# aapdo/M3ViT

Measured on AMD Instinct MI355X. Metric: images/sec fwd+bwd ViT-S/16 MoE(E=16,k=4) 224^2 bs=128, higher is better.
Workload: dtype f16; 1 GPU; configs[1]: ViT-Small/16 + MoE E=16 top-k=4 multi_gate, synthetic 224x224; batch_per_gpu=128, global_batch=128, task_passes=2, launch=hipGraph replay (one linear graph per task pass and stream), routing=deterministic (std=0), task_streams=2, wgrad_streams=0, activation_checkpointing=False, parallelism=single, full=False

## Files before the change

### m3vit_amd/csrc/wgrad_dev.h

```cpp
#pragma once
#include "common.h"
#include <type_traits>

namespace m3 {

constexpr int WG_T = 128;
constexpr int WG_ROWS = 64;
constexpr int WG_THREADS = 256;
constexpr int BG_T = 256, BG_THREADS = 512, BG_RS = 512;

constexpr int WG_MULTI = 8;

struct WgradRdProb {
  const float *ws; float *dW; const float *bws; float *db;
  int64_t e4; int32_t b4;
  int32_t nbw;
  int32_t first;
  int32_t beta;
};

struct WgradDev {
  const char *dC; int64_t lddc_b; const int32_t *c_row_idx;
  int32_t c_row_div; const float *c_row_scale;
  int32_t a_row_sh, c_row_sh;
  const char *A; int64_t lda_b; const int32_t *a_row_idx; int32_t a_row_div;
  int64_t M; int32_t N; int32_t K; int32_t G;
  const int32_t *group_offsets;
  int32_t splits;
  float *ws;
  float *bias_ws;
  int32_t tiles_k;
  int32_t chunk_rows;
  int32_t rd_blocks, rd_zslices;
  int32_t rd_nbx, rd_nbw;
  int32_t rd_cols;
  const float *rd_ws; int32_t rd_splits; int64_t rd_e4;
  const int32_t *rd_off; int32_t rd_G, rd_chunk;
  float *rd_dW; int32_t rd_beta;
  const float *rd_bws; int64_t rd_b4; float *rd_db; int32_t rd_beta_db;
  int32_t rd_n;
  WgradRdProb rd_tab0, rd_tab1, rd_tab2, rd_tab3, rd_tab4, rd_tab5, rd_tab6, rd_tab7;
  float *direct_dW; float *direct_db; int32_t direct_beta, direct_beta_db;
  int32_t lpt;
};

__device__ __forceinline__ void wgrad_store_tile(const WgradDev &p, const f32x4 (&acc)[4][4], int64_t slab_id, int g, int n0, int k0,
                                                 int wr, int wc, int li, int lg) {
  float *out = p.direct_dW ? p.direct_dW + (int64_t)g * p.N * p.K : p.ws + slab_id * (int64_t)p.N * p.K;
  const bool add = p.direct_dW && p.direct_beta;
#pragma unroll
  for (int ni = 0; ni < 4; ++ni) {
    const int n = n0 + wc * 64 + ni * 16 + li;
    if (n >= p.N) continue;
    f32x4 old[4];
    if (add) {
#pragma unroll
      for (int ki = 0; ki < 4; ++ki) {
        const int k = k0 + wr * 64 + ki * 16 + 4 * lg;
        old[ki] = k < p.K ? *(const f32x4 *)(out + (int64_t)n * p.K + k) : f32x4{0.f, 0.f, 0.f, 0.f};
      }
    }
#pragma unroll
    for (int ki = 0; ki < 4; ++ki) {
      const int k = k0 + wr * 64 + ki * 16 + 4 * lg;
      if (k >= p.K) continue;
      *(f32x4 *)(out + (int64_t)n * p.K + k) = add ? acc[ki][ni] + old[ki] : acc[ki][ni];
    }
  }
}
__device__ __forceinline__ void wgrad_store_bias(const WgradDev &p, float v, int64_t slab_id, int g, int n) {
  if (p.direct_db) {
    float *d = p.direct_db + (int64_t)g * p.N + n;
    *d = p.direct_beta_db ? *d + v : v;
  } else {
    p.bias_ws[slab_id * p.N + n] = v;
  }
}

__host__ __device__ __forceinline__ int wgrad_units_of_group(int rows, int chunk) { return (rows + chunk - 1) / chunk; }
__host__ __device__ __forceinline__ void wgrad_unit_rows(int rows, int n, int j, int &begin, int &end) {
  const int per = ((rows + n - 1) / n + WG_ROWS - 1) / WG_ROWS * WG_ROWS;
  begin = j * per;
  end = begin + per < rows ? begin + per : rows;
}

__device__ __forceinline__ void wgrad_unit_scan(const int32_t *off, int G, int chunk, int lane, int &rows, int &n, int &first) {
  rows = lane < G ? off[lane + 1] - off[lane] : 0;
  n = wgrad_units_of_group(rows, chunk);
  int incl = n;
#pragma unroll
  for (int d = 1; d < 64; d <<= 1) {
    const int t = __shfl_up(incl, d, 64);
    if (lane >= d) incl += t;
  }
  first = incl - n;
}

__device__ __forceinline__ bool wgrad_unit(const int32_t *off, int G, int chunk, int lin, int tiles, int lane, int &tile,
                                           int &u, int &g, int64_t &r0, int64_t &r1) {
  int rows, n, first;
  wgrad_unit_scan(off, G, chunk, lane, rows, n, first);
  const int units = __shfl(first + n, 63, 64);
  if (lin >= units * tiles) return false;
  const int log_id = xcd_remap(lin, units * tiles);
  tile = log_id % tiles;
  u = log_id / tiles;
  const unsigned long long m = __ballot(u >= first && u < first + n);
  g = __ffsll((long long)m) - 1;
  rows = __shfl(rows, g, 64); n = __shfl(n, g, 64); first = __shfl(first, g, 64);
  int b, e;
  wgrad_unit_rows(rows, n, u - first, b, e);
  r0 = (int64_t)off[g] + b;
  r1 = (int64_t)off[g] + e;
  return true;
}

__device__ __forceinline__ int wgrad_lpt_group(const int32_t *off, int G, int u, int lane) {
  if (G > 64 || (G & 7)) return u;
  const int cnt = lane < G ? off[lane + 1] - off[lane] : -1;
  int rank = 0;
  for (int j = 0; j < G; ++j) {
    const int cj = __shfl(cnt, j, 64);
    rank += (cj > cnt || (cj == cnt && j < lane)) ? 1 : 0;
  }
  const int per = G >> 3;
  const int want = 8 * (u % per) + u / per;
  const unsigned long long m = __ballot(lane < G && rank == want);
  return __ffsll((long long)m) - 1;
}

struct WgradProb {
  const char *dC; int64_t lddc_b; const char *A; int64_t lda_b;
  float *ws; float *bias_ws;
  int32_t N, K, tiles_k;
  int32_t first;
};
struct WgradMultiDev {
  WgradDev d;
  WgradProb tab0, tab1, tab2, tab3, tab4, tab5, tab6, tab7;
};

typedef __fp16 fp16x4_t __attribute__((__vector_size__(4 * sizeof(__fp16))));

__device__ __forceinline__ f32x4 wgrad_sum_slabs(const f32x4 *w, int64_t elems4, int lo, int hi, f32x4 s) {
  int sp = lo;
  for (; sp + 8 <= hi; sp += 8) {
    f32x4 v[8];
#pragma unroll
    for (int j = 0; j < 8; ++j) v[j] = w[(int64_t)(sp + j) * elems4];
#pragma unroll
    for (int j = 0; j < 8; ++j) s += v[j];
  }
  for (; sp < hi; ++sp) s += w[(int64_t)sp * elems4];
  return s;
}
__device__ __forceinline__ void wgrad_reduce_block(int64_t blk, int tid, const float *ws, int splits, int64_t elems4, float *dW,
                                                   int beta, int nb_w, const float *bias_ws, int64_t belems4, float *db, int beta_db,
                                                   int cols) {
  if (blk >= nb_w) {
    blk -= nb_w; ws = bias_ws; elems4 = belems4; dW = db; beta = beta_db;
  }
  if (cols == 256) {
    const int64_t i = blk * 256 + tid;
    if (i >= elems4) return;
    f32x4 s = beta ? ((const f32x4 *)dW)[i] : f32x4{0.f, 0.f, 0.f, 0.f};
    ((f32x4 *)dW)[i] = wgrad_sum_slabs((const f32x4 *)ws + i, elems4, 0, splits, s);
    return;
  }
  __shared__ f32x4 spart[3][64];
  const int col = tid & 63, part = tid >> 6;
  const int64_t i = blk * 64 + col;
  const bool in = i < elems4;
  f32x4 s = f32x4{0.f, 0.f, 0.f, 0.f};
  if (in) {
    if (part == 0 && beta) s = ((const f32x4 *)dW)[i];
    s = wgrad_sum_slabs((const f32x4 *)ws + i, elems4, splits * part / 4, splits * (part + 1) / 4, s);
  }
  if (part > 0) spart[part - 1][col] = s;
  __syncthreads();
  if (part == 0 && in) {
    s += spart[0][col]; s += spart[1][col]; s += spart[2][col];
    ((f32x4 *)dW)[i] = s;
  }
}

__device__ __forceinline__ void wgrad_reduce_grouped_block(int64_t blk, int g, int tid, const float *ws, const int32_t *off, int G,
                                                           int chunk, int64_t elems4, float *dW, int beta, int nb_w,
                                                           const float *bias_ws, int64_t belems4, float *db, int beta_db) {
  if (blk >= nb_w) {
    blk -= nb_w; ws = bias_ws; elems4 = belems4; dW = db; beta = beta_db;
  }
  const int64_t i = blk * 256 + tid;
  int rows, n, first;
  wgrad_unit_scan(off, G, chunk, tid & 63, rows, n, first);
  n = __shfl(n, g, 64); first = __shfl(first, g, 64);
  if (i >= elems4) return;
  f32x4 *out = (f32x4 *)dW + (int64_t)g * elems4 + i;
  f32x4 s = beta ? *out : f32x4{0.f, 0.f, 0.f, 0.f};
  const f32x4 *w = (const f32x4 *)ws + (int64_t)first * elems4 + i;
  int u = 0;
  for (; u + 8 <= n; u += 8) {
    f32x4 v[8];
#pragma unroll
    for (int j = 0; j < 8; ++j) v[j] = w[(int64_t)(u + j) * elems4];
#pragma unroll
    for (int j = 0; j < 8; ++j) s += v[j];
  }
  if (u + 4 <= n) {
    f32x4 v[4];
#pragma unroll
    for (int j = 0; j < 4; ++j) v[j] = w[(int64_t)(u + j) * elems4];
#pragma unroll
    for (int j = 0; j < 4; ++j) s += v[j];
    u += 4;
  }
  if (u + 2 <= n) {
    const f32x4 v0 = w[(int64_t)u * elems4], v1 = w[(int64_t)(u + 1) * elems4];
    s += v0; s += v1;
    u += 2;
  }
  if (u < n) s += w[(int64_t)u * elems4];
  *out = s;
}

__device__ __forceinline__ bool wgrad_ride_along(const WgradDev &p, int tid, int &bz, int &gz) {
  bz = blockIdx.z; gz = gridDim.z;
  if (p.rd_blocks <= 0) return false;
  if (bz < p.rd_zslices) {
    const int rid = blockIdx.x + (int)gridDim.x * (blockIdx.y + (int)gridDim.y * bz);
    if (rid < p.rd_blocks) {
      const int g = rid / p.rd_nbx, bx = rid - g * p.rd_nbx;
      if (p.rd_n > 1) {
        const float *ws = p.rd_tab0.ws, *bws = p.rd_tab0.bws;
        float *dW = p.rd_tab0.dW, *db = p.rd_tab0.db;
        int64_t e4 = p.rd_tab0.e4;
        int b4 = p.rd_tab0.b4, nbw = p.rd_tab0.nbw, first = p.rd_tab0.first, beta = p.rd_tab0.beta;
#define M3_RD_FROM(j)                                                                                                   \
  {                                                                                                                     \
    const float *ws_ = p.rd_tab##j.ws, *bws_ = p.rd_tab##j.bws;                                                         \
    float *dW_ = p.rd_tab##j.dW, *db_ = p.rd_tab##j.db;                                                                 \
    const int64_t e4_ = p.rd_tab##j.e4;                                                                                 \
    const int b4_ = p.rd_tab##j.b4, nbw_ = p.rd_tab##j.nbw, first_ = p.rd_tab##j.first, beta_ = p.rd_tab##j.beta;       \
    const bool h_ = rid >= first_;                                                                                      \
    ws = h_ ? ws_ : ws; bws = h_ ? bws_ : bws; dW = h_ ? dW_ : dW; db = h_ ? db_ : db; e4 = h_ ? e4_ : e4;              \
    b4 = h_ ? b4_ : b4; nbw = h_ ? nbw_ : nbw; first = h_ ? first_ : first; beta = h_ ? beta_ : beta;                   \
  }
        static_assert(WG_MULTI == 8, "one M3_RD_FROM per entry");
        M3_RD_FROM(1) M3_RD_FROM(2) M3_RD_FROM(3) M3_RD_FROM(4) M3_RD_FROM(5) M3_RD_FROM(6) M3_RD_FROM(7)
#undef M3_RD_FROM
        wgrad_reduce_block(rid - first, tid, ws, p.rd_splits, e4, dW, beta & 1, nbw, bws, b4, db, beta >> 1, p.rd_cols);
      } else if (p.rd_chunk)
        wgrad_reduce_grouped_block(bx, g, tid, p.rd_ws, p.rd_off, p.rd_G, p.rd_chunk, p.rd_e4, p.rd_dW, p.rd_beta, p.rd_nbw,
                                   p.rd_bws, p.rd_b4, p.rd_db, p.rd_beta_db);
      else
        wgrad_reduce_block(bx, tid, p.rd_ws, p.rd_splits, p.rd_e4, p.rd_dW, p.rd_beta, p.rd_nbw, p.rd_bws, p.rd_b4, p.rd_db,
                           p.rd_beta_db, p.rd_cols);
    }
    return true;
  }
  bz -= p.rd_zslices; gz -= p.rd_zslices;
  return false;
}

template <typename T> __device__ __forceinline__ u32x4 scale_chunk(u32x4 v, float s);
template <> __device__ __forceinline__ u32x4 scale_chunk<half_t>(u32x4 v, float s) {
  f16x8 f = __builtin_bit_cast(f16x8, v);
#pragma unroll
  for (int j = 0; j < 8; ++j) f[j] = (half_t)((float)f[j] * s);
  return __builtin_bit_cast(u32x4, f);
}
template <> __device__ __forceinline__ u32x4 scale_chunk<bf16_t>(u32x4 v, float s) {
  bf16x8 f = __builtin_bit_cast(bf16x8, v);
#pragma unroll
  for (int j = 0; j < 8; ++j) f[j] = (bf16_t)((float)f[j] * s);
  return __builtin_bit_cast(u32x4, f);
}
template <> __device__ __forceinline__ u32x4 scale_chunk<float>(u32x4 v, float s) {
  return __builtin_bit_cast(u32x4, __builtin_bit_cast(f32x4, v) * s);
}

__device__ __forceinline__ f16x8 wgrad_tr16_frag(const char *p0, const char *p1) {
  typedef __attribute__((address_space(3))) fp16x4_t lds_h4;
  const fp16x4_t lo = __builtin_amdgcn_ds_read_tr16_b64_v4f16((lds_h4 *)p0);
  const fp16x4_t hi = __builtin_amdgcn_ds_read_tr16_b64_v4f16((lds_h4 *)p1);
  f16x8 f;
  f[0] = (half_t)lo[0]; f[1] = (half_t)lo[1]; f[2] = (half_t)lo[2]; f[3] = (half_t)lo[3];
  f[4] = (half_t)hi[0]; f[5] = (half_t)hi[1]; f[6] = (half_t)hi[2]; f[7] = (half_t)hi[3];
  return f;
}
template <typename T> __device__ __forceinline__ float wgrad_colsum8(const typename Mma<T>::frag &f, float a) {
  typedef T t2 __attribute__((ext_vector_type(2)));
  if constexpr (sizeof(T) == 4) {
    return a + ((f[0] + f[1]) + (f[2] + f[3]));
  } else {
#pragma unroll
    for (int j = 0; j < 4; ++j) {
      const t2 pr = t2{f[2 * j], f[2 * j + 1]};
      if constexpr (std::is_same<T, half_t>::value)
        a = __builtin_amdgcn_fdot2(pr, t2{(T)1, (T)1}, a, false);
      else if constexpr (std::is_same<T, bf16_t>::value)
        a = __builtin_amdgcn_fdot2_f32_bf16(pr, t2{(T)1.f, (T)1.f}, a, false);
    }
    return a;
  }
}
__device__ __forceinline__ f16x8 wgrad_factor_f16x8(f32x4 s0, f32x4 s1) {
  return f16x8{(half_t)s0[0], (half_t)s0[1], (half_t)s0[2], (half_t)s0[3], (half_t)s1[0], (half_t)s1[1], (half_t)s1[2], (half_t)s1[3]};
}

enum WgradKernel { WGRAD_STAGED, WGRAD_DMA, WGRAD_BIG, WGRAD_SKINNY };

template <typename T> constexpr int wgrad_dtype_of = std::is_same<T, half_t>::value ? M3_F16 : std::is_same<T, bf16_t>::value ? M3_BF16 : M3_F32;
template <typename Fam, typename T, int I = 0, typename F> static inline void wgrad_each_flags(F &f) {
  if constexpr (I < 8) {
    constexpr bool GC = (I & 1) != 0, GA = (I & 2) != 0, SC = (I & 4) != 0;
    if (const void *k = Fam::template instance<T, GC, GA, SC>()) f(wgrad_dtype_of<T>, GC, GA, SC, k);
    wgrad_each_flags<Fam, T, I + 1>(f);
  }
}
template <typename Fam, typename F> static inline void wgrad_each_instance(F f) {
  wgrad_each_flags<Fam, half_t>(f); wgrad_each_flags<Fam, bf16_t>(f); wgrad_each_flags<Fam, float>(f);
}
template <typename Fam>
static inline int wgrad_launch_instance(int dtype, bool gc, bool ga, bool sc, dim3 grid, dim3 block, size_t lds, WgradDev d, hipStream_t s) {
  const void *kernel = nullptr;
  wgrad_each_instance<Fam>([&](int dt, bool c, bool a, bool f, const void *k) { if (dt == dtype && c == gc && a == ga && f == sc) kernel = k; });
  M3_REQUIRE(kernel, "m3_wgrad_tn: no kernel instance for dtype %d, gathers (%d, %d), per-row factor %d", dtype, gc, ga, sc);
  void *args[] = {&d};
  (void)hipLaunchKernel(kernel, grid, block, args, lds, s);
  return check_launch("m3_wgrad_tn");
}

int launch_wgrad_staged(int dtype, bool gc, bool ga, bool sc, dim3 grid, const WgradDev &d, hipStream_t s);
int launch_wgrad_dma(int dtype, bool gc, bool ga, bool sc, dim3 grid, const WgradDev &d, hipStream_t s);
int launch_wgrad_big(int dtype, bool gc, bool ga, bool sc, dim3 grid, const WgradDev &d, hipStream_t s);
int launch_wgrad_multi(int dtype, dim3 grid, const WgradMultiDev &d, hipStream_t s);

}
```

### m3vit_amd/csrc/wgrad_staged.hip

```cpp
#include "wgrad_dev.h"

namespace m3 {

template <typename T> struct WgLds;
template <> struct WgLds<half_t> { static constexpr int STRIDE = 288; static constexpr int ROWS = 32; };
template <> struct WgLds<bf16_t> { static constexpr int STRIDE = 288; static constexpr int ROWS = 32; };
template <> struct WgLds<float> { static constexpr int STRIDE = 528; static constexpr int ROWS = 32; };

template <typename T>
__device__ __forceinline__ typename Mma<T>::frag read_tr_frag(const char *base, int rb, int col, int li, int lg);

template <>
__device__ __forceinline__ f16x8 read_tr_frag<half_t>(const char *base, int rb, int col, int li, int lg) {
  const char *p0 = base + (rb + 4 * lg + (li >> 2)) * WgLds<half_t>::STRIDE + (col + 4 * (li & 3)) * 2;
  const char *p1 = p0 + 16 * WgLds<half_t>::STRIDE;
  return wgrad_tr16_frag(p0, p1);
}

template <>
__device__ __forceinline__ bf16x8 read_tr_frag<bf16_t>(const char *base, int rb, int col, int li, int lg) {
  return __builtin_bit_cast(bf16x8, read_tr_frag<half_t>(base, rb, col, li, lg));
}

template <>
__device__ __forceinline__ f32x4 read_tr_frag<float>(const char *base, int rb, int col, int li, int lg) {
  const char *p = base + (rb + 4 * lg) * WgLds<float>::STRIDE + (col + li) * 4;
  f32x4 f;
  f[0] = *(const float *)(p);
  f[1] = *(const float *)(p + WgLds<float>::STRIDE);
  f[2] = *(const float *)(p + 2 * WgLds<float>::STRIDE);
  f[3] = *(const float *)(p + 3 * WgLds<float>::STRIDE);
  return f;
}

#ifdef M3_WGRAD_STAMPS
constexpr int WTSTAMP_WGS = 128, WTSTAMP_N = 2 + 4 * 80;
__device__ unsigned long long g_wtn_stamps[WTSTAMP_WGS][WTSTAMP_N];
#define WT_STAMP(i)                                                                                                   \
  do {                                                                                                                \
    const int wg_ = blockIdx.y + gridDim.y * blockIdx.z;                                                              \
    if (threadIdx.x == 0 && blockIdx.x == 0 && wg_ < WTSTAMP_WGS && (i) < WTSTAMP_N)                                  \
      g_wtn_stamps[wg_][(i)] = __builtin_amdgcn_s_memtime();                                                          \
  } while (0)
#else
#define WT_STAMP(i) do { } while (0)
#endif

template <typename T, bool GC, bool GA, bool SC>
__device__ __forceinline__ void wgrad_tile_loop(const WgradDev &p, int tile, int g, int64_t slab_id, int64_t r0, int64_t r1,
                                                int64_t s_begin, int nst) {
  typedef Mma<T> MM;
  typedef typename MM::frag frag;
  constexpr int ES = (int)sizeof(T);
  constexpr int EPC = 16 / ES;
  constexpr int STRIDE = WgLds<T>::STRIDE;
  constexpr int ROWS = WgLds<T>::ROWS;
  constexpr int CPR = WG_T * ES / 16;
  constexpr int NLD = ROWS * CPR / WG_THREADS;
  constexpr int RSTEP = WG_THREADS / CPR;
  constexpr int OPB = ROWS * STRIDE;
  constexpr int KCH = ROWS / MM::KC;

  extern __shared__ __attribute__((aligned(16))) char smem[];

  const int tid = threadIdx.x;
  const int lane = tid & 63, wave = tid >> 6;
  const int li = lane & 15, lg = lane >> 4;
  const int wr = wave >> 1, wc = wave & 1;

  const int tn = tile / p.tiles_k, tk = tile - tn * p.tiles_k;
  const int n0 = tn * WG_T, k0 = tk * WG_T;

  f32x4 acc[4][4];
#pragma unroll
  for (int a = 0; a < 4; ++a)
#pragma unroll
    for (int b = 0; b < 4; ++b) acc[a][b] = f32x4{0.f, 0.f, 0.f, 0.f};

  const int srow = tid / CPR, c = tid - srow * CPR;
  int ncol = n0 + c * EPC, kcol = k0 + c * EPC;
  if (ncol > p.N - EPC) ncol = p.N - EPC;
  if (kcol > p.K - EPC) kcol = p.K - EPC;
  const char *c_base = p.dC + (int64_t)ncol * ES;
  const char *a_base = p.A + (int64_t)kcol * ES;
  const int st_off = srow * STRIDE + c * 16;
  const uint32_t ldc = (uint32_t)p.lddc_b, lda = (uint32_t)p.lda_b;
  const uint32_t rbase = (uint32_t)(r0 + s_begin * ROWS + srow);
  const uint32_t rend = (uint32_t)r1;

  auto row_of = [&](int step, int i) -> uint32_t {
    const uint32_t m = rbase + (uint32_t)(step * ROWS + i * RSTEP);
    return m < rend ? m : rend - 1;
  };
  auto load_index = [&](int step, int32_t(&ic)[NLD], int32_t(&ia)[NLD]) {
#pragma unroll
    for (int i = 0; i < NLD; ++i) {
      const uint32_t m = row_of(step, i);
      if (GC) ic[i] = p.c_row_idx[m];
      if (GA) ia[i] = p.a_row_idx[m];
    }
  };
  auto load_global = [&](int step, const int32_t(&ic)[NLD], const int32_t(&ia)[NLD], u32x4(&rc)[NLD], u32x4(&ra)[NLD],
                         float(&rs)[NLD]) {
#pragma unroll
    for (int i = 0; i < NLD; ++i) {
      const uint32_t m = row_of(step, i);
      const uint32_t cr = GC ? (uint32_t)div_by(ic[i], p.c_row_div, p.c_row_sh) : m;
      const uint32_t ar = GA ? (uint32_t)div_by(ia[i], p.a_row_div, p.a_row_sh) : m;
      rc[i] = *(const u32x4 *)(c_base + (uint64_t)cr * ldc);
      ra[i] = *(const u32x4 *)(a_base + (uint64_t)ar * lda);
      if (SC) rs[i] = p.c_row_scale[ic[i]];
    }
  };
  auto store_lds = [&](int buf, int step, const u32x4(&rc)[NLD], const u32x4(&ra)[NLD], const float(&rs)[NLD]) {
    char *base = smem + buf * (2 * OPB) + st_off;
#pragma unroll
    for (int i = 0; i < NLD; ++i) {
      const bool ok = rbase + (uint32_t)(step * ROWS + i * RSTEP) < rend;
      const u32x4 cv = SC ? scale_chunk<T>(rc[i], rs[i]) : rc[i];
      *(u32x4 *)(base + i * RSTEP * STRIDE) = ok ? cv : u32x4{0u, 0u, 0u, 0u};
      *(u32x4 *)(base + i * RSTEP * STRIDE + OPB) = ok ? ra[i] : u32x4{0u, 0u, 0u, 0u};
    }
  };
  const bool do_bias = (p.bias_ws || p.direct_db) && tk == 0 && wr == 0;
  f32x4 acc_b[4];
#pragma unroll
  for (int i = 0; i < 4; ++i) acc_b[i] = f32x4{0.f, 0.f, 0.f, 0.f};
  frag ones;
#pragma unroll
  for (int j = 0; j < MM::EPL; ++j) ones[j] = (T)1.0f;

  auto compute = [&](int buf) {
    const char *sC = smem + buf * (2 * OPB), *sA = sC + OPB;
#pragma unroll
    for (int kc = 0; kc < KCH; ++kc) {
      frag fk[4], fn[4];
#pragma unroll
      for (int i = 0; i < 4; ++i) {
        fk[i] = read_tr_frag<T>(sA, kc * MM::KC, wr * 64 + i * 16, li, lg);
        fn[i] = read_tr_frag<T>(sC, kc * MM::KC, wc * 64 + i * 16, li, lg);
      }
#pragma unroll
      for (int ki = 0; ki < 4; ++ki)
#pragma unroll
        for (int ni = 0; ni < 4; ++ni) acc[ki][ni] = MM::mma(fk[ki], fn[ni], acc[ki][ni]);
      if (do_bias) {
#pragma unroll
        for (int ni = 0; ni < 4; ++ni) acc_b[ni] = MM::mma(ones, fn[ni], acc_b[ni]);
      }
    }
  };

  WT_STAMP(0);
  if (nst > 0) {
    const int last = nst - 1;
    auto cl = [&](int s_) { return s_ < last ? s_ : last; };
    u32x4 rc0[NLD], ra0[NLD], rc1[NLD], ra1[NLD];
    float sc0[NLD], sc1[NLD];
    int32_t ic0[NLD], ia0[NLD], ic1[NLD], ia1[NLD];
    auto fetch = [&](int ds, int32_t(&ic)[NLD], int32_t(&ia)[NLD], u32x4(&rc)[NLD], u32x4(&ra)[NLD], float(&rs)[NLD],
                     int32_t(&jc)[NLD], int32_t(&ja)[NLD]) {
      load_global(ds, ic, ia, rc, ra, rs);
#if defined(M3_WGRAD_STAMPS) && defined(M3_WGRAD_TN_INDEX_BEHIND)
      load_index(cl(ds + 1), jc, ja);
#else
      load_index(cl(ds + 2), ic, ia);
#endif
    };
    load_index(0, ic0, ia0);
    load_index(cl(1), ic1, ia1);
    load_global(0, ic0, ia0, rc1, ra1, sc1);
    load_index(cl(2), ic0, ia0);
    load_global(cl(1), ic1, ia1, rc0, ra0, sc0);
    load_index(cl(3), ic1, ia1);
    store_lds(0, 0, rc1, ra1, sc1);
    __syncthreads();
    WT_STAMP(1);
    int t = 0;
    for (; t + 3 < nst; t += 2) {
      fetch(t + 2, ic0, ia0, rc1, ra1, sc1, ic1, ia1);
      __builtin_amdgcn_sched_barrier(0);
      WT_STAMP(2 + 4 * t);
      compute(0);
      WT_STAMP(3 + 4 * t);
      store_lds(1, t + 1, rc0, ra0, sc0);
      WT_STAMP(4 + 4 * t);
      __syncthreads();
      WT_STAMP(5 + 4 * t);
      fetch(t + 3, ic1, ia1, rc0, ra0, sc0, ic0, ia0);
      __builtin_amdgcn_sched_barrier(0);
      WT_STAMP(6 + 4 * t);
      compute(1);
      WT_STAMP(7 + 4 * t);
      store_lds(0, t + 2, rc1, ra1, sc1);
      WT_STAMP(8 + 4 * t);
      __syncthreads();
      WT_STAMP(9 + 4 * t);
    }
    const int rem = nst - t;
    if (rem == 3) {
      load_global(t + 2, ic0, ia0, rc1, ra1, sc1);
      compute(0);
      store_lds(1, t + 1, rc0, ra0, sc0);
      __syncthreads();
      compute(1);
      store_lds(0, t + 2, rc1, ra1, sc1);
      __syncthreads();
      compute(0);
    } else if (rem == 2) {
      compute(0);
      store_lds(1, t + 1, rc0, ra0, sc0);
      __syncthreads();
      compute(1);
    } else {
      compute(0);
    }
  }

  if (do_bias && lg == 0) {
#pragma unroll
    for (int ni = 0; ni < 4; ++ni) {
      const int n = n0 + wc * 64 + ni * 16 + li;
      if (n < p.N) wgrad_store_bias(p, acc_b[ni][0], slab_id, g, n);
    }
  }
  wgrad_store_tile(p, acc, slab_id, g, n0, k0, wr, wc, li, lg);
}

template <typename T, bool GC, bool GA, bool SC = false>
__global__ __launch_bounds__(WG_THREADS, 2) void wgrad_tn_kernel(const WgradDev p) {
  constexpr int ROWS = WgLds<T>::ROWS;
  const int tid = threadIdx.x;
  const int lane = tid & 63;

  const int tiles = gridDim.x;
  int bz, gz;
  if (wgrad_ride_along(p, tid, bz, gz)) return;
  const int lin = blockIdx.x + tiles * (blockIdx.y + gridDim.y * bz);
  int tile, gs, g, sp, nst;
  int64_t r0, r1, s_begin;
  if (p.chunk_rows) {
    if (!wgrad_unit(p.group_offsets, p.G, p.chunk_rows, lin, tiles, lane, tile, gs, g, r0, r1)) return;
    sp = gs; s_begin = 0;
    nst = (int)((r1 - r0 + ROWS - 1) / ROWS);
  } else {
    const int log_id = xcd_remap(lin, tiles * gridDim.y * gz);
    tile = log_id % tiles; gs = log_id / tiles;
    g = gs % (int)gridDim.y; sp = gs / (int)gridDim.y;
    if (p.group_offsets && p.lpt) g = wgrad_lpt_group(p.group_offsets, p.G, g, lane);
    if (p.group_offsets) { r0 = p.group_offsets[g]; r1 = p.group_offsets[g + 1]; }
    else { r0 = 0; r1 = p.M; }
    const int64_t nsteps_all = (r1 - r0 + ROWS - 1) / ROWS;
    const int64_t per = (nsteps_all + p.splits - 1) / p.splits;
    s_begin = (int64_t)sp * per;
    int64_t s_end = s_begin + per;
    if (s_end > nsteps_all) s_end = nsteps_all;
    nst = (int)(s_end > s_begin ? s_end - s_begin : 0);
  }
  const int64_t slab_id = p.chunk_rows ? (int64_t)sp : (int64_t)sp * p.G + g;
  wgrad_tile_loop<T, GC, GA, SC>(p, tile, g, slab_id, r0, r1, s_begin, nst);
}

struct WgStaged {
  template <typename T, bool GC, bool GA, bool SC> static const void *instance() {
    if constexpr (!SC || GC) return (const void *)wgrad_tn_kernel<T, GC, GA, SC>;
    else return nullptr;
  }
};

int launch_wgrad_staged(int dtype, bool gc, bool ga, bool sc, dim3 grid, const WgradDev &d, hipStream_t s) {
  const size_t lds16 = 4 * WgLds<half_t>::ROWS * WgLds<half_t>::STRIDE, lds32 = 4 * WgLds<float>::ROWS * WgLds<float>::STRIDE;
  static bool attr_set = false;
  if (!attr_set) {
    wgrad_each_instance<WgStaged>([&](int dt, bool, bool, bool, const void *k) {
      (void)hipFuncSetAttribute(k, hipFuncAttributeMaxDynamicSharedMemorySize, (int)(dt == M3_F32 ? lds32 : lds16));
    });
    attr_set = true;
  }
  return wgrad_launch_instance<WgStaged>(dtype, gc, ga, sc, grid, dim3(WG_THREADS), dtype == M3_F32 ? lds32 : lds16, d, s);
}

}

#ifdef M3_WGRAD_STAMPS
extern "C" int m3_debug_wtn_stamps(unsigned long long *dst, int wgs, int clear) {
  using namespace m3;
  if (wgs > WTSTAMP_WGS) wgs = WTSTAMP_WGS;
  const size_t bytes = (size_t)wgs * WTSTAMP_N * sizeof(unsigned long long);
  if (dst && hipMemcpyFromSymbol(dst, HIP_SYMBOL(g_wtn_stamps), bytes) != hipSuccess) return M3_ERR_LAUNCH;
  if (clear) {
    void *sym = nullptr;
    if (hipGetSymbolAddress(&sym, HIP_SYMBOL(g_wtn_stamps)) != hipSuccess || hipMemset(sym, 0, sizeof(g_wtn_stamps)) != hipSuccess) return M3_ERR_LAUNCH;
  }
  return M3_OK;
}
#endif
```

Measured before the change: 7743 images/s.

## Stage gather row indices in an LDS table and advance ungathered row pointers incrementally

The staged weight-gradient kernel used to load row indices and scale factors from global memory every step, per thread and per loaded row. It now fetches them cooperatively in 256-row pieces, applies the divisor once, and writes them to a double-buffered LDS table. Later steps read this table, spreading the piece loads across a four-pair-of-steps schedule. For ungathered operands it advances precomputed pointers instead of recomputing row addresses and clamps. This cuts dependent global index latency and address arithmetic in the inner loop, at the cost of extra LDS, which may affect occupancy, and more code specialisation.

```diff
diff --git a/m3vit_amd/csrc/wgrad_dev.h b/m3vit_amd/csrc/wgrad_dev.h
--- a/m3vit_amd/csrc/wgrad_dev.h
+++ b/m3vit_amd/csrc/wgrad_dev.h
@@ -8,6 +8,9 @@
 constexpr int WG_ROWS = 64;
 constexpr int WG_THREADS = 256;
 constexpr int BG_T = 256, BG_THREADS = 512, BG_RS = 512;
+
+constexpr int WG_TAB_ROWS = WG_THREADS;
+constexpr int WG_TAB_BYTES = 3 * 2 * WG_TAB_ROWS * 4;
 
 constexpr int WG_MULTI = 8;
 
diff --git a/m3vit_amd/csrc/wgrad_staged.hip b/m3vit_amd/csrc/wgrad_staged.hip
--- a/m3vit_amd/csrc/wgrad_staged.hip
+++ b/m3vit_amd/csrc/wgrad_staged.hip
@@ -85,38 +85,83 @@
   const char *a_base = p.A + (int64_t)kcol * ES;
   const int st_off = srow * STRIDE + c * 16;
   const uint32_t ldc = (uint32_t)p.lddc_b, lda = (uint32_t)p.lda_b;
-  const uint32_t rbase = (uint32_t)(r0 + s_begin * ROWS + srow);
+  const uint32_t rfirst = (uint32_t)(r0 + s_begin * ROWS);
+  const uint32_t rbase = rfirst + (uint32_t)srow;
   const uint32_t rend = (uint32_t)r1;
 
   auto row_of = [&](int step, int i) -> uint32_t {
     const uint32_t m = rbase + (uint32_t)(step * ROWS + i * RSTEP);
     return m < rend ? m : rend - 1;
   };
-  auto load_index = [&](int step, int32_t(&ic)[NLD], int32_t(&ia)[NLD]) {
+  constexpr int TMASK = 2 * WG_TAB_ROWS - 1;
+  static_assert(WG_TAB_ROWS % ROWS == 0 && WG_TAB_ROWS / ROWS == 8, "a piece is four pairs of steps");
+  uint32_t *tab_c = (uint32_t *)(smem + 2 * (2 * OPB));
+  float *tab_f = (float *)(tab_c + 2 * WG_TAB_ROWS);
+  uint32_t *tab_a = (uint32_t *)(tab_f + 2 * WG_TAB_ROWS);
+  auto tab_request = [&](int piece, int32_t &xc, int32_t &xa) {
+    uint32_t m = rfirst + (uint32_t)(piece * WG_TAB_ROWS + tid);
+    m = m < rend ? m : rend - 1;
+    if (GC) xc = p.c_row_idx[m];
+    if (GA) xa = p.a_row_idx[m];
+  };
+  auto tab_factor = [&](int32_t xc, float &f) {
+    if (SC) f = p.c_row_scale[xc];
+  };
+  auto tab_write_rows = [&](int piece, int32_t xc, int32_t xa) {
+    const int e = (piece & 1) * WG_TAB_ROWS + tid;
+    if (GC) tab_c[e] = (uint32_t)div_by(xc, p.c_row_div, p.c_row_sh);
+    if (GA) tab_a[e] = (uint32_t)div_by(xa, p.a_row_div, p.a_row_sh);
+  };
+  auto tab_write_factor = [&](int piece, float f) {
+    if (SC) tab_f[(piece & 1) * WG_TAB_ROWS + tid] = f;
+  };
+  auto tab_rows = [&](int step, uint32_t(&nc)[NLD], uint32_t(&na)[NLD]) {
 #pragma unroll
     for (int i = 0; i < NLD; ++i) {
-      const uint32_t m = row_of(step, i);
-      if (GC) ic[i] = p.c_row_idx[m];
-      if (GA) ia[i] = p.a_row_idx[m];
-    }
-  };
-  auto load_global = [&](int step, const int32_t(&ic)[NLD], const int32_t(&ia)[NLD], u32x4(&rc)[NLD], u32x4(&ra)[NLD],
-                         float(&rs)[NLD]) {
+      const int e = (step * ROWS + srow + i * RSTEP) & TMASK;
+      if (GC) nc[i] = tab_c[e];
+      if (GA) na[i] = tab_a[e];
+    }
+  };
+  auto tab_factors = [&](int step, float(&rs)[NLD]) {
+#pragma unroll
+    for (int i = 0; i < NLD; ++i)
+      if (SC) rs[i] = tab_f[(step * ROWS + srow + i * RSTEP) & TMASK];
+  };
+  typedef std::false_type any_step;
+  typedef std::true_type whole_step;
+  const char *pc[NLD], *pa[NLD];
+  const uint64_t bump_c = (uint64_t)ROWS * ldc, bump_a = (uint64_t)ROWS * lda;
+  auto point_at = [&](int step) {
 #pragma unroll
     for (int i = 0; i < NLD; ++i) {
-      const uint32_t m = row_of(step, i);
-      const uint32_t cr = GC ? (uint32_t)div_by(ic[i], p.c_row_div, p.c_row_sh) : m;
-      const uint32_t ar = GA ? (uint32_t)div_by(ia[i], p.a_row_div, p.a_row_sh) : m;
-      rc[i] = *(const u32x4 *)(c_base + (uint64_t)cr * ldc);
-      ra[i] = *(const u32x4 *)(a_base + (uint64_t)ar * lda);
-      if (SC) rs[i] = p.c_row_scale[ic[i]];
-    }
-  };
-  auto store_lds = [&](int buf, int step, const u32x4(&rc)[NLD], const u32x4(&ra)[NLD], const float(&rs)[NLD]) {
+      const uint32_t m = rbase + (uint32_t)(step * ROWS + i * RSTEP);
+      pc[i] = c_base + (uint64_t)m * ldc;
+      pa[i] = a_base + (uint64_t)m * lda;
+    }
+  };
+  auto load_global = [&](auto whole, int step, const uint32_t(&nc)[NLD], const uint32_t(&na)[NLD], u32x4(&rc)[NLD],
+                         u32x4(&ra)[NLD]) {
+    constexpr bool W = decltype(whole)::value;
+#pragma unroll
+    for (int i = 0; i < NLD; ++i) {
+      const char *cp, *ap;
+      if constexpr (GC) cp = c_base + (uint64_t)nc[i] * ldc;
+      else if constexpr (W) { cp = pc[i]; pc[i] += bump_c; }
+      else cp = c_base + (uint64_t)row_of(step, i) * ldc;
+      if constexpr (GA) ap = a_base + (uint64_t)na[i] * lda;
+      else if constexpr (W) { ap = pa[i]; pa[i] += bump_a; }
+      else ap = a_base + (uint64_t)row_of(step, i) * lda;
+      rc[i] = *(const u32x4 *)cp;
+      ra[i] = *(const u32x4 *)ap;
+    }
+  };
+  auto store_lds = [&](auto whole, int buf, int step, const u32x4(&rc)[NLD], const u32x4(&ra)[NLD], const float(&rs)[NLD]) {
+    constexpr bool W = decltype(whole)::value;
     char *base = smem + buf * (2 * OPB) + st_off;
 #pragma unroll
     for (int i = 0; i < NLD; ++i) {
-      const bool ok = rbase + (uint32_t)(step * ROWS + i * RSTEP) < rend;
+      const bool ok = W || rbase + (uint32_t)(step * ROWS + i * RSTEP) < rend;
       const u32x4 cv = SC ? scale_chunk<T>(rc[i], rs[i]) : rc[i];
       *(u32x4 *)(base + i * RSTEP * STRIDE) = ok ? cv : u32x4{0u, 0u, 0u, 0u};
       *(u32x4 *)(base + i * RSTEP * STRIDE + OPB) = ok ? ra[i] : u32x4{0u, 0u, 0u, 0u};
@@ -156,60 +201,103 @@
     const int last = nst - 1;
     auto cl = [&](int s_) { return s_ < last ? s_ : last; };
     u32x4 rc0[NLD], ra0[NLD], rc1[NLD], ra1[NLD];
-    float sc0[NLD], sc1[NLD];
-    int32_t ic0[NLD], ia0[NLD], ic1[NLD], ia1[NLD];
-    auto fetch = [&](int ds, int32_t(&ic)[NLD], int32_t(&ia)[NLD], u32x4(&rc)[NLD], u32x4(&ra)[NLD], float(&rs)[NLD],
-                     int32_t(&jc)[NLD], int32_t(&ja)[NLD]) {
-      load_global(ds, ic, ia, rc, ra, rs);
-#if defined(M3_WGRAD_STAMPS) && defined(M3_WGRAD_TN_INDEX_BEHIND)
-      load_index(cl(ds + 1), jc, ja);
-#else
-      load_index(cl(ds + 2), ic, ia);
-#endif
+    uint32_t nc[NLD] = {}, na[NLD] = {};
+    float rs[NLD] = {};
+    constexpr bool AHEAD = ES == 2 || (GC && GA);
+    auto fetch = [&](auto whole, int ds, u32x4(&rc)[NLD], u32x4(&ra)[NLD]) {
+      if constexpr (!AHEAD) tab_rows(ds, nc, na);
+      load_global(whole, ds, nc, na, rc, ra);
+      if constexpr (AHEAD) tab_rows(cl(ds + 1), nc, na);
     };
-    load_index(0, ic0, ia0);
-    load_index(cl(1), ic1, ia1);
-    load_global(0, ic0, ia0, rc1, ra1, sc1);
-    load_index(cl(2), ic0, ia0);
-    load_global(cl(1), ic1, ia1, rc0, ra0, sc0);
-    load_index(cl(3), ic1, ia1);
-    store_lds(0, 0, rc1, ra1, sc1);
+    auto store_step = [&](int buf, int step, const u32x4(&rc)[NLD], const u32x4(&ra)[NLD]) {
+      tab_factors(step, rs);
+      store_lds(any_step(), buf, step, rc, ra, rs);
+    };
+    int32_t ti_c = 0, ti_a = 0;
+    float tf = 0.f;
+    if constexpr (GC || GA) {
+      int32_t t0c = 0, t0a = 0;
+      tab_request(0, t0c, t0a);
+      tab_request(1, ti_c, ti_a);
+      tab_write_rows(0, t0c, t0a);
+      tab_write_rows(1, ti_c, ti_a);
+      float f0 = 0.f;
+      tab_factor(t0c, f0);
+      tab_factor(ti_c, tf);
+      __syncthreads();
+      tab_rows(0, nc, na);
+      fetch(any_step(), 0, rc1, ra1);
+      fetch(any_step(), cl(1), rc0, ra0);
+      if constexpr (SC) {
+        tab_write_factor(0, f0);
+        tab_write_factor(1, tf);
+        __syncthreads();
+      }
+    } else {
+      fetch(any_step(), 0, rc1, ra1);
+      fetch(any_step(), cl(1), rc0, ra0);
+    }
+    store_step(0, 0, rc1, ra1);
     __syncthreads();
     WT_STAMP(1);
-    int t = 0;
-    for (; t + 3 < nst; t += 2) {
-      fetch(t + 2, ic0, ia0, rc1, ra1, sc1, ic1, ia1);
+    auto two_steps = [&](auto whole, auto stage, int t) {
+      constexpr int ST = decltype(stage)::value;
+      const int piece = (t >> 3) + 2, place = (t >> 1) & 3;
+      if (ST == 1 || (ST < 0 && place == 0)) tab_request(piece, ti_c, ti_a);
+      if (ST == 2 || (ST < 0 && place == 1)) tab_factor(ti_c, tf);
+      fetch(whole, t + 2, rc1, ra1);
+      tab_factors(t + 1, rs);
       __builtin_amdgcn_sched_barrier(0);
       WT_STAMP(2 + 4 * t);
       compute(0);
       WT_STAMP(3 + 4 * t);
-      store_lds(1, t + 1, rc0, ra0, sc0);
+      store_lds(whole, 1, t + 1, rc0, ra0, rs);
       WT_STAMP(4 + 4 * t);
       __syncthreads();
       WT_STAMP(5 + 4 * t);
-      fetch(t + 3, ic1, ia1, rc0, ra0, sc0, ic0, ia0);
+      if (ST == 3 || (ST < 0 && place == 3)) {
+        tab_write_rows(piece, ti_c, ti_a);
+        tab_write_factor(piece, tf);
+      }
+      fetch(whole, t + 3, rc0, ra0);
+      tab_factors(t + 2, rs);
       __builtin_amdgcn_sched_barrier(0);
       WT_STAMP(6 + 4 * t);
       compute(1);
       WT_STAMP(7 + 4 * t);
-      store_lds(0, t + 2, rc1, ra1, sc1);
+      store_lds(whole, 0, t + 2, rc1, ra1, rs);
       WT_STAMP(8 + 4 * t);
       __syncthreads();
       WT_STAMP(9 + 4 * t);
-    }
+    };
+    typedef std::integral_constant<int, 0> no_stage;
+    int t = 0;
+    if constexpr (ES == 2) point_at(2);
+    if constexpr ((GC || GA) && ES == 2) {
+      for (; t + 10 < nst; t += 8) {
+        two_steps(whole_step(), std::integral_constant<int, 1>(), t);
+        two_steps(whole_step(), std::integral_constant<int, 2>(), t + 2);
+        two_steps(whole_step(), no_stage(), t + 4);
+        two_steps(whole_step(), std::integral_constant<int, 3>(), t + 6);
+      }
+    }
+    if constexpr (ES == 2)
+      for (; t + 4 < nst; t += 2) two_steps(whole_step(), no_stage(), t);
+    typedef std::integral_constant<int, (GC || GA) && ES != 2 ? -1 : 0> tail_stage;
+    for (; t + 3 < nst; t += 2) two_steps(any_step(), tail_stage(), t);
     const int rem = nst - t;
     if (rem == 3) {
-      load_global(t + 2, ic0, ia0, rc1, ra1, sc1);
-      compute(0);
-      store_lds(1, t + 1, rc0, ra0, sc0);
+      fetch(any_step(), t + 2, rc1, ra1);
+      compute(0);
+      store_step(1, t + 1, rc0, ra0);
       __syncthreads();
       compute(1);
-      store_lds(0, t + 2, rc1, ra1, sc1);
+      store_step(0, t + 2, rc1, ra1);
       __syncthreads();
       compute(0);
     } else if (rem == 2) {
       compute(0);
-      store_lds(1, t + 1, rc0, ra0, sc0);
+      store_step(1, t + 1, rc0, ra0);
       __syncthreads();
       compute(1);
     } else {
@@ -270,14 +358,16 @@
 
 int launch_wgrad_staged(int dtype, bool gc, bool ga, bool sc, dim3 grid, const WgradDev &d, hipStream_t s) {
   const size_t lds16 = 4 * WgLds<half_t>::ROWS * WgLds<half_t>::STRIDE, lds32 = 4 * WgLds<float>::ROWS * WgLds<float>::STRIDE;
+  static_assert(2 * (4 * WgLds<float>::ROWS * WgLds<float>::STRIDE + WG_TAB_BYTES) <= 160 * 1024, "two workgroups per CU");
   static bool attr_set = false;
   if (!attr_set) {
     wgrad_each_instance<WgStaged>([&](int dt, bool, bool, bool, const void *k) {
-      (void)hipFuncSetAttribute(k, hipFuncAttributeMaxDynamicSharedMemorySize, (int)(dt == M3_F32 ? lds32 : lds16));
+      (void)hipFuncSetAttribute(k, hipFuncAttributeMaxDynamicSharedMemorySize, (int)((dt == M3_F32 ? lds32 : lds16) + WG_TAB_BYTES));
     });
     attr_set = true;
   }
-  return wgrad_launch_instance<WgStaged>(dtype, gc, ga, sc, grid, dim3(WG_THREADS), dtype == M3_F32 ? lds32 : lds16, d, s);
+  const size_t lds = (dtype == M3_F32 ? lds32 : lds16) + (gc || ga ? WG_TAB_BYTES : 0);
+  return wgrad_launch_instance<WgStaged>(dtype, gc, ga, sc, grid, dim3(WG_THREADS), lds, d, s);
 }
 
 }
```

New measurement: 7864 images/s (median of 6 runs). 1.02x the previous value.
